# pmgbergen/porepy

Measured on AMD Instinct MI355X. Metric: cells/sec MPFA assemble+solve, 3D unstructured grid, higher is better.
Workload: dtype f64

## Files before the change

### include/porefv.h

```cpp
#ifndef POREFV_H
#define POREFV_H

#include <stddef.h>
#include <stdint.h>

#ifdef __cplusplus
extern "C" {
#endif

typedef struct pfv_ctx pfv_ctx;

typedef enum {
  PFV_OK = 0,
  PFV_ERR_SINGULAR = 1,
  PFV_ERR_CELL_SHAPE = 2,
  PFV_ERR_HIP = 3,
  PFV_ERR_ARGUMENT = 4,
  PFV_ERR_UNSUPPORTED = 5,
  PFV_ERR_NOT_CONVERGED = 6
} pfv_status;

enum {
  PFV_MAT_FLUX = 0,
  PFV_MAT_BOUND_FLUX = 1,
// ... 90 lines not shown
  int64_t sweep_launches;
  double sweep_order_ms;
  int64_t sweep_direct_steps;
  int64_t sweep_direct_fallbacks;
  int64_t transport_multi_components;
  int64_t transport_multi_direct_steps;
  int64_t transport_multi_fallback_components;
  double transport_nl_ms;
  int64_t transport_nl_steps;
  int64_t transport_nl_core_iterations;
  int64_t transport_nl_components;
  double transport_react_ms;
  int64_t transport_react_steps;
  int64_t transport_react_core_iterations;
  int64_t transport_react_components;
  double transport_adjoint_ms;
  int64_t transport_adjoint_steps;
  int64_t transport_adjoint_core_iterations;
  int64_t amg_ap_nnz;
  double transport_react_adjoint_ms;
  int64_t transport_react_adjoint_steps;
  int64_t transport_react_adjoint_core_iterations;
  int64_t amg_galerkin_ap;
} pfv_stats;

pfv_status pfv_create(int device, pfv_ctx** out);
void pfv_destroy(pfv_ctx* h);
const char* pfv_last_error(pfv_ctx* h);
int pfv_is_device_build(void);

pfv_status pfv_set_grid(pfv_ctx* h, int nd, int64_t nc, int64_t nf, int64_t nn,
                        const double* nodes, const int32_t* cf_indptr,
                        const int32_t* cf_indices, const int8_t* cf_sign,
                        const int32_t* fn_indptr, const int32_t* fn_indices,
                        const double* face_normals, const double* face_centers,
                        const double* cell_centers, const double* face_areas);

pfv_status pfv_mpfa_set_params(pfv_ctx* h, const double* perm_33n, const uint8_t* bc_flags,
                               const double* robin_weight, double eta,
                               const double* eta_subface);

pfv_status pfv_mpfa_set_permeability(pfv_ctx* h, const double* perm_33n);

#define PFV_AD_WANT_FLUX_JACOBIAN 1u
pfv_status pfv_mpfa_ad_flux_system(pfv_ctx* h, const double* p, const double* dk_dp, const double* bc_values,
                                   const double* vector_source, const double* source, double* flux_out,
// ... 212 lines not shown
```

### porepy_amd/_lib.py

```python
from __future__ import annotations

import ctypes as C
import os

import numpy as np

_HERE = os.path.dirname(os.path.abspath(__file__))
DEFAULT_LIBRARY = os.path.join(_HERE, "csrc", "libporefv_hip.so")

MAT_FLUX, MAT_BOUND_FLUX, MAT_BOUND_PRESSURE_CELL, MAT_BOUND_PRESSURE_FACE = 0, 1, 2, 3
MAT_VECTOR_SOURCE, MAT_BOUND_PRESSURE_VECTOR_SOURCE, MAT_SYSTEM = 4, 5, 6
MAT_STRESS, MAT_BOUND_STRESS, MAT_BOUND_DISPLACEMENT_CELL, MAT_BOUND_DISPLACEMENT_FACE, MAT_MECH_SYSTEM = 7, 8, 9, 10, 11
MAT_USER_SYSTEM = 12
MAT_FLUX_JACOBIAN = 13
MAT_UPWIND, MAT_UPWIND_RHS_DIR, MAT_UPWIND_RHS_NEU, MAT_TRANSPORT_SYSTEM = 14, 15, 16, 17
MAT_ADVDIFF_SYSTEM = 18
BC_DIR, BC_NEU, BC_ROB, BC_INTERNAL = 1, 2, 4, 8
SOLVE_CG, SOLVE_BICGSTAB, SOLVE_GMRES = 0, 1, 2
PRECOND_JACOBI, PRECOND_AMG, PRECOND_BLOCK, PRECOND_AMG_NNS, PRECOND_SWEEP = 0, 1, 2, 3, 4
FLUXFN_LINEAR, FLUXFN_COREY, FLUXFN_TABLE = 0, 1, 2
DISCR_REBUILD_TOPOLOGY, DISCR_SKIP_VECTOR_SOURCE = 1, 2

STATUS_NAMES = {
    0: "ok", 1: "singular local system", 2: "unsupported cell shape", 3: "HIP error",
# ... 40 lines not shown
                ("win_reused", C.c_int64), ("amg_filter_layout", C.c_int64),
                ("solve_launches", C.c_int64), ("amg_setup_launches", C.c_int64), ("node_redo", C.c_int64),
                ("symbolic_reused", C.c_int64), ("amg_stale_rematches", C.c_int64),
                ("mpsa_contrast_regions", C.c_int64), ("mpsa_max_contrast", C.c_double), ("assemble_positions_kept", C.c_int64),
                ("pipeline_runs", C.c_int64), ("amg_nns_modes", C.c_int64),
                ("face_flux_ms", C.c_double), ("upwind_ms", C.c_double), ("transport_assemble_ms", C.c_double),
                ("transport_advance_ms", C.c_double), ("transport_iterations", C.c_int64),
                ("transport_gmres_retries", C.c_int64),
                ("advdiff_assemble_ms", C.c_double), ("advdiff_advance_ms", C.c_double),
                ("advdiff_iterations", C.c_int64), ("advdiff_precond_fallbacks", C.c_int64),
                ("advdiff_gmres_retries", C.c_int64),
                ("sweep_levels", C.c_int64), ("sweep_core_cells", C.c_int64), ("sweep_launches", C.c_int64),
                ("sweep_order_ms", C.c_double), ("sweep_direct_steps", C.c_int64),
                ("sweep_direct_fallbacks", C.c_int64),
                ("transport_multi_components", C.c_int64), ("transport_multi_direct_steps", C.c_int64),
                ("transport_multi_fallback_components", C.c_int64),
                ("transport_nl_ms", C.c_double), ("transport_nl_steps", C.c_int64),
                ("transport_nl_core_iterations", C.c_int64), ("transport_nl_components", C.c_int64),
                ("transport_react_ms", C.c_double), ("transport_react_steps", C.c_int64),
                ("transport_react_core_iterations", C.c_int64), ("transport_react_components", C.c_int64),
                ("transport_adjoint_ms", C.c_double), ("transport_adjoint_steps", C.c_int64),
                ("transport_adjoint_core_iterations", C.c_int64), ("amg_ap_nnz", C.c_int64),
                ("transport_react_adjoint_ms", C.c_double), ("transport_react_adjoint_steps", C.c_int64),
                ("transport_react_adjoint_core_iterations", C.c_int64), ("amg_galerkin_ap", C.c_int64)]

    def as_dict(self):
        return {n: getattr(self, n) for n, _ in self._fields_}


HALO_FN = C.CFUNCTYPE(C.c_int, C.c_void_p, C.c_void_p, C.c_void_p)
ALLREDUCE_FN = C.CFUNCTYPE(C.c_int, C.c_void_p, C.c_void_p, C.c_int, C.c_void_p)


SENDRECV_FN = C.CFUNCTYPE(C.c_int, C.c_void_p, C.c_int, C.POINTER(C.c_int32), C.c_void_p, C.POINTER(C.c_int64),
                          C.c_void_p, C.POINTER(C.c_int64), C.c_void_p)
ALLGATHER_FN = C.CFUNCTYPE(C.c_int, C.c_void_p, C.c_void_p, C.c_void_p, C.c_int64, C.c_void_p)


class ShardHooks(C.Structure):
    _fields_ = [("exchange_halo", HALO_FN), ("allreduce_sum", ALLREDUCE_FN), ("user", C.c_void_p),
                ("sendrecv", SENDRECV_FN), ("allgather", ALLGATHER_FN)]


class PorefvError(RuntimeError):
    def __init__(self, status: int, message: str):
        super().__init__(f"porefv status {status} ({STATUS_NAMES.get(status, '?')}): {message}")
        self.status = status
# ... 1546 lines not shown
```

### porepy_amd/csrc/amg.inc

```

namespace pfv {

constexpr int kAmgDenseMax = 1024;
constexpr int kAmgCoarseTargetDefault = 160;
constexpr int kAmgMaxLevels = 14;
constexpr int64_t kAmgWTopRows = 600000;
constexpr int kAmgFilterPermilBlock = 50;
constexpr int kAmgFilterPermil = 30;
constexpr int kAmgRounds = 4;
constexpr int kAmgPasses = 3;
constexpr int kAmgGentleCells = 400000;
constexpr int kGalEpl = 8;
constexpr int kGalMaxMembers = 16;
constexpr int64_t kAmgGatherRowsDefault = 32768;

struct AmgSwitches {
  int bs = 1;
  bool omega_auto = false;
  bool safe_rows = true;
  double omega = 0.95, alpha = 1.5;
  int omega_power_steps = 10;
  double omega_sigma = 1.8;
  int passes = kAmgPasses;
  bool passes_coarse_set = false;
  int passes_coarse_raw = -1;
  int rounds = kAmgRounds, rounds_raw = kAmgRounds;
  int strength_neg = 0;
  bool fp32 = true;
  double filter_theta = 0.0;
  int coarse_target = kAmgCoarseTargetDefault;
  bool gamma_set = false;
  int gamma_raw = 0;
  int gamma_levels = 1;
  int64_t fuse_rows = 30000;
  bool fuse_cycle = true;
  bool restrict_lanes = true;
  bool reuse = true, reuse_dist = true, reuse_rebuilt = true;
  int reuse_dist_min_rows = 500000;
  bool members_reuse = true, sizes_reuse = true;
  bool filter_smooth = true, rowmax_reuse = true, filter_layout_reuse = true, skip_moved_digest = true;
  bool galerkin_batched = true, filter_unroll = true, dense_lds = true;
  int64_t gather_rows = kAmgGatherRowsDefault;
  bool post_ap = true;
  bool galerkin_ap = true;
};

static AmgSwitches amg_read_switches(int bs) {
  auto given = [](const char* name, int& v) {
    const char* e = std::getenv(name);
    if (e) v = std::atoi(e);
    return e != nullptr;
  };
  auto on = [](const char* name, int dflt) { return env_int(name, dflt) != 0; };
  AmgSwitches w;
  w.bs = bs;
  w.safe_rows = on("PFV_AMG_SAFE_ROWS", bs == 1 ? 1 : 0);
  int omega_pct = w.safe_rows ? 95 : 80;
  w.omega_auto = !given("PFV_AMG_OMEGA_PCT", omega_pct) && on("PFV_AMG_OMEGA_AUTO", 0);
  w.omega = 0.01 * omega_pct;
  w.alpha = 0.01 * env_int("PFV_AMG_ALPHA_PCT", 150);
  w.omega_power_steps = std::max(2, std::min(30, env_int("PFV_AMG_OMEGA_POWER_STEPS", 10)));
  w.omega_sigma = 0.01 * env_int("PFV_AMG_OMEGA_RHO_PCT", 180);
  w.passes = std::max(1, std::min(6, env_int("PFV_AMG_PASSES", kAmgPasses)));
  w.passes_coarse_set = given("PFV_AMG_PASSES_COARSE", w.passes_coarse_raw);
// ... 1 lines not shown
  w.rounds = std::max(1, std::min(12, w.rounds_raw));
  w.strength_neg = env_int("PFV_AMG_STRENGTH_NEG", 0);
  w.fp32 = on("PFV_AMG_FP32", 1);
  w.filter_theta = 0.001 * env_int(bs == 1 ? "PFV_AMG_FILTER_PERMIL" : "PFV_AMG_FILTER_PERMIL_BLOCK",
                                   bs == 1 ? kAmgFilterPermil : kAmgFilterPermilBlock);
  w.coarse_target = std::max(1, std::min(kAmgDenseMax, env_int("PFV_AMG_COARSE_TARGET", kAmgCoarseTargetDefault)));
  w.gamma_set = given("PFV_AMG_GAMMA", w.gamma_raw);
  w.gamma_levels = env_int("PFV_AMG_GAMMA_LEVELS", 1);
  w.fuse_rows = env_int("PFV_AMG_FUSE_ROWS", 30000);
  w.fuse_cycle = on("PFV_AMG_FUSE_CYCLE", 1);
  w.restrict_lanes = on("PFV_AMG_RESTRICT_LANES", bs == 1 ? 1 : 0);
  w.reuse = on("PFV_AMG_REUSE", 1);
  w.reuse_dist = on("PFV_AMG_REUSE_DIST", 1);
  w.reuse_rebuilt = on("PFV_AMG_REUSE_REBUILT", 1);
  w.reuse_dist_min_rows = env_int("PFV_AMG_REUSE_DIST_MIN_ROWS", 500000);
  w.members_reuse = on("PFV_AMG_MEMBERS_REUSE", 1);
  w.sizes_reuse = on("PFV_AMG_SIZES_REUSE", 1);
  w.filter_smooth = on("PFV_AMG_FILTER_SMOOTH", 1);
  w.rowmax_reuse = on("PFV_AMG_ROWMAX_REUSE", 1);
  w.filter_layout_reuse = on("PFV_AMG_FILTER_LAYOUT_REUSE", 1);
  w.skip_moved_digest = on("PFV_AMG_SKIP_MOVED_DIGEST", 1);
  w.galerkin_batched = on("PFV_AMG_GALERKIN_BATCHED", 1);
  w.filter_unroll = on("PFV_AMG_FILTER_UNROLL", 1);
  w.dense_lds = on("PFV_AMG_DENSE_LDS", 1);
  w.gather_rows = std::max<int64_t>(1, env_int("PFV_AMG_GATHER_ROWS", (int)kAmgGatherRowsDefault));
  w.post_ap = on("PFV_AMG_POST_AP", 1);
  w.galerkin_ap = on("PFV_AMG_GALERKIN_AP", 1);
  return w;
}

static int64_t amg_maps_cfg(const AmgSwitches& w) {
  return ((((int64_t)w.passes * 16 + w.rounds_raw) * 16 + w.passes_coarse_raw + 1) * 4 + w.strength_neg) * 65536 +
         w.coarse_target * 8 + w.bs + (int64_t)(1000.0 * w.filter_theta + 0.5) * (int64_t(1) << 40);
}
static int amg_maps_tag(const AmgSwitches& w) { return w.rounds_raw * 64 + w.passes_coarse_raw + 1; }

struct AmgLevel {
  int64_t n = 0;
  int64_t m = 0;
  const CsrPattern* P = nullptr;
  const double* val = nullptr;
  CsrPattern P_own;
  Buf<double> val_own;
  Buf<float> val32;
  const float* v32 = nullptr;
  WinCsr win_own;
// ... 65 lines not shown
  Amg();
  ~Amg();
  std::unique_ptr<AmgDist> dist;
  bool no_filter = false;
  int64_t finest_cells_parent = 0;
  std::vector<std::unique_ptr<AmgLevel>> lev;
  size_t nlev = 0;
  AmgWork wk;
  int bs = 1;
  AmgSwitches sw;
  int passes = kAmgPasses;
  double omega = 0.8, alpha = 1.5;
  bool omega_auto = true;
  Buf<double> pw_a, pw_b, pw_zero, pw_part;
  Buf<double> dense;
  unsigned long long filt_layout_for = 0;
  bool filt_layout_stable = false;
  CsrPattern filtP;
  Buf<double> filtV;
  double filter_theta = 0.0;
  int64_t filt_nnz = 0;
  bool filter_level0 = false;
  WinCsr filt_win;
  struct GalSizes { int64_t ncr, annz, nnz; int maxcap; };
  std::vector<GalSizes> gal_sizes;
  unsigned long long gal_for_sum = 0;
  bool gal_use = false;
  size_t gal_k = 0;
  int gal_route = 0;
  unsigned long long filt_win_sum = 0;
  bool maps_ok = false, reused = false;
  int64_t maps_n = -1, maps_nnz = -1, maps_cfg = 0;
  unsigned long long maps_sum = 0, maps_epoch = 0;
  int maps_tag = 0;
  int iters_fresh = -1;
  int method_fresh = -1;
  double rtol_fresh = 0.0;
  int64_t stale_rematches = 0;
  void note_iterations(int iterations, double rtol, int method, bool converged) {
    if (!valid) return;
    if (!reused) {
      iters_fresh = converged ? iterations : -1;
      rtol_fresh = rtol;
      method_fresh = method;
    } else if (iters_fresh > 0 && rtol == rtol_fresh && method == method_fresh &&
               (!converged || (double)iterations > 1.3 * (double)iters_fresh + 1.0)) {
// ... 394 lines not shown
  std::swap(a.nnz, b.nnz);
  std::swap(a.max_row, b.max_row);
  a.indptr.swap(b.indptr);
  a.indices.swap(b.indices);
}

static unsigned long long amg_pattern_checksum(pfv_ctx_impl& c, AmgWork& wk, const CsrPattern& P) {
  if (&P == &c.pat_A && c.pat_A_checksum != 0 && c.have_symbolic) return c.pat_A_checksum;
  return read_scalar<unsigned long long>(c.stream, launch_pattern_checksum(c, wk.csum, P));
}

struct AmgBlockStrength {
  const int32_t* ip;
  const double* val;
  int bs;
  PFV_HD double operator()(int64_t r, int kb) const {
    const int64_t i = r / bs;
    double sw = 0.0;
    for (int a = 0; a < bs; ++a) sw += fabs(val[ip[i * bs + a] + kb * bs + a]);
    return sw;
  }
};

#ifndef PFV_EMULATE
constexpr int kFilterUnroll = 5;

static void amg_filter_count_scalar(stream_t s, int64_t n, const int32_t* ip, const int32_t* ix, const double* val,
                                    const double* rmax, double theta, int32_t* cnt) {
  wave_for<16>(s, n, 16, PFV_LAMBDA(const WaveCtx& w) {
    const int64_t r = w.item;
    const int p0 = ip[r], nb = ip[r + 1] - p0;
    const double mi = rmax[r];
    int kept = 0;
    for (int c0 = 0; c0 < nb; c0 += kFilterUnroll * 16) {
      int cj[kFilterUnroll];
      double v[kFilterUnroll], rm[kFilterUnroll];
#pragma unroll
      for (int u = 0; u < kFilterUnroll; ++u) {
        const int kb = c0 + u * 16 + w.lane;
        const bool live = kb < nb;
        cj[u] = live ? ix[p0 + kb] : -1;
        v[u] = live ? val[p0 + kb] : 0.0;
      }
#pragma unroll
      for (int u = 0; u < kFilterUnroll; ++u) rm[u] = cj[u] >= 0 ? rmax[cj[u]] : 0.0;
#pragma unroll
// ... 55 lines not shown
          fv[o] = v[u];
          if (isdiag) { od = o; dv = v[u]; }
        }
        base += total;
      }
    }
    lump[w.lane] = mylump;
    w.lsync();
    if (spec && w.lane0() && base != room) atomic_max_i32(bad, 1);
    const unsigned long long has = __ballot(od >= 0);
    const bool any_diag = ((has >> sh) & 0xffffull) != 0ull;
    if (od >= 0) {
      double sum = 0.0;
      for (int l = 0; l < 16; ++l) sum += lump[l];
      const double d = dv + sum;
      fv[od] = d;
      if (dinv_out) dinv_out[r] = d != 0.0 ? 1.0 / d : 0.0;
    } else if (!any_diag && w.lane0() && dinv_out) {
      dinv_out[r] = 0.0;
    }
    w.lsync();
  });
}
#endif

static void amg_filter(pfv_ctx_impl& c, const AmgSwitches& sw, const CsrPattern& A, const double* val, double theta,
                       CsrPattern& F, Buf<double>& FV, AmgWork& wk, int bs = 1,
                       const std::function<void(double*)>& fill_halo = nullptr, const double* rmax_given = nullptr,
                       double* dinv_out = nullptr, bool same_layout_expected = false, bool* layout_unchanged = nullptr) {
  stream_t s = c.stream;
  const int64_t n = A.nrows;
  const int32_t* ip = A.indptr;
  const int32_t* ix = A.indices;
  int32_t* cnt = wk.cnt.ensure(n + 1);
  int64_t* pos = wk.pos.ensure(n + 2);
  double* rmax = wk.tval.ensure(std::max<int64_t>(std::max(n, A.ncols), 1));
  constexpr int kMaxBs = 4;
  if (bs > kMaxBs) throw Error(PFV_ERR_UNSUPPORTED, "AMG filter: block size above 4");
  const AmgBlockStrength strength{ip, val, bs};
  const bool have_rmax = rmax_given != nullptr && bs == 1 && !fill_halo;
  if (have_rmax) be_d2d(rmax, rmax_given, sizeof(double) * (size_t)n, s);
  else
  wave_for<16>(s, n, 16 * sizeof(double) + 16, PFV_LAMBDA(const WaveCtx& w) {
    const int64_t r = w.item;
    const int64_t i = r / bs;
    double* mx = reinterpret_cast<double*>(w.lds);
    const int p0 = ip[r], nb = (ip[r + 1] - p0) / bs;
    double m = 0.0;
    PFV_LANES(kb, nb) {
      if (ix[p0 + kb * bs] / bs != (int32_t)i) m = fmax(m, strength(r, kb));
    }
    mx[w.lane] = m;
    w.lsync();
    if (w.lane0()) {
      double mm = 0.0;
      for (int l = 0; l < w.width; ++l) mm = fmax(mm, mx[l]);
      rmax[r] = mm;
    }
    w.lsync();
  });
  if (fill_halo) fill_halo(rmax);
  const bool spec = same_layout_expected && F.nrows == n && F.ncols == A.ncols && F.nnz > 0 && F.indptr.p != nullptr;
  int32_t* bad = c.status.ensure(16) + 12;
  if (spec) be_memset(bad, 0, sizeof(int32_t), s);
#ifndef PFV_EMULATE
  const bool fast = bs == 1 && sw.filter_unroll;
#else
  const bool fast = false;
#endif
  if (!spec) {
#ifndef PFV_EMULATE
  if (fast) amg_filter_count_scalar(s, n, ip, ix, val, rmax, theta, cnt);
  else
#endif
  wave_for<16>(s, n, 16 * sizeof(int32_t) + 16, PFV_LAMBDA(const WaveCtx& w) {
    const int64_t r = w.item;
    const int64_t i = r / bs;
    int32_t* ct = reinterpret_cast<int32_t*>(w.lds);
    const int p0 = ip[r], nb = (ip[r + 1] - p0) / bs;
    const double mi = rmax[r];
    int kept = 0;
    PFV_LANES(kb, nb) {
      const int cj = ix[p0 + kb * bs] / bs;
      if (cj == (int32_t)i || strength(r, kb) >= theta * fmin(mi, rmax[(int64_t)cj * bs])) ++kept;
    }
#ifndef PFV_EMULATE
    (void)ct;
    kept += __shfl_xor(kept, 8, 16);
    kept += __shfl_xor(kept, 4, 16);
    kept += __shfl_xor(kept, 2, 16);
    kept += __shfl_xor(kept, 1, 16);
    if (w.lane0()) cnt[r] = kept * bs;
#else
    ct[w.lane] = kept;
    w.lsync();
    if (w.lane0()) {
      int tot = 0;
      for (int l = 0; l < w.width; ++l) tot += ct[l];
      cnt[r] = tot * bs;
    }
    w.lsync();
#endif
  });
  exclusive_scan<int32_t, int64_t>(s, c.scratch, cnt, pos, (size_t)n);
  }
  const bool compare = !spec && layout_unchanged != nullptr && F.nrows == n && F.nnz > 0 && F.indptr.p != nullptr;
  if (!spec) {
    be_memset(pos + n + 1, 0, sizeof(int64_t), s);
    if (compare) {
      const int32_t* old = F.indptr.p;
      parallel_for(s, n, PFV_LAMBDA(int64_t r) {
        if (old[r + 1] - old[r] != cnt[r]) pos[n + 1] = 1;
      });
    }
  }
  int64_t tail[2] = {F.nnz, 0};
  if (!spec) be_d2h(tail, pos + n, 2 * sizeof(int64_t), s);
  if (layout_unchanged) *layout_unchanged = spec || (compare && tail[1] == 0 && tail[0] == F.nnz);
  const int64_t nnz = tail[0];
  F.nrows = n;
  F.ncols = A.ncols;
  F.nnz = nnz;
  F.max_row = A.max_row;
  int32_t* fp = F.indptr.ensure(n + 1);
  int32_t* fx = F.indices.ensure(std::max<int64_t>(nnz, 1));
  double* fv = FV.ensure(std::max<int64_t>(nnz, 1));
  if (!spec) parallel_for(s, n + 1, PFV_LAMBDA(int64_t q) { fp[q] = (int32_t)pos[q]; });
#ifndef PFV_EMULATE
  if (fast) amg_filter_compact_scalar(s, n, ip, ix, val, rmax, theta, fp, fx, fv, dinv_out, spec, bad);
  else
#endif
  wave_for<16>(s, n, (16 + 1) * kMaxBs * sizeof(double) + 20 * sizeof(int32_t) + 16, PFV_LAMBDA(const WaveCtx& w) {
    const int64_t r = w.item;
    const int64_t i = r / bs;
    double* lump = reinterpret_cast<double*>(w.lds);
    double* dblk = lump + 16 * kMaxBs;
    int32_t* flag = reinterpret_cast<int32_t*>(dblk + kMaxBs);
    const int p0 = ip[r], nb = (ip[r + 1] - p0) / bs;
    const double mi = rmax[r];
    if (w.lane0()) flag[16] = -1;
    w.lsync();
    double mylump[kMaxBs];
    for (int b = 0; b < kMaxBs; ++b) mylump[b] = 0.0;
    int base = fp[r];
    for (int c0 = 0; c0 < nb; c0 += w.width) {
      const int kb = c0 + w.lane;
      bool keep = false;
      const bool live = kb < nb;
      bool isdiag = false;
      if (live) {
        const int cj = ix[p0 + kb * bs] / bs;
        isdiag = cj == (int32_t)i;
// ... 36 lines not shown
      base += total * bs;
      w.lsync();
    }
    for (int b = 0; b < bs; ++b) lump[w.lane * kMaxBs + b] = mylump[b];
    w.lsync();
    if (spec && w.lane0() && base != fp[r + 1]) atomic_max_i32(bad, 1);
    if (w.lane0()) {
      const int od = flag[16];
      if (od >= 0) {
        for (int b = 0; b < bs; ++b) {
          double sum = 0.0;
          for (int l = 0; l < w.width; ++l) sum += lump[l * kMaxBs + b];
          const double dv = dblk[b] + sum;
          fv[od + b] = dv;
          if (dinv_out && b == (int)(r - i * bs)) dinv_out[r] = dv != 0.0 ? 1.0 / dv : 0.0;
        }
      } else if (dinv_out) {
        dinv_out[r] = 0.0;
      }
    }
    w.lsync();
  });
  c.stats.amg_filter_layout = spec ? 1 : 0;
  if (spec && read_scalar<int32_t>(s, bad) != 0) {
    amg_filter(c, sw, A, val, theta, F, FV, wk, bs, fill_halo, rmax_given, dinv_out, false, nullptr);
    c.stats.amg_filter_layout = 2;
    if (layout_unchanged) *layout_unchanged = false;
  }
}

static void amg_estimate_omegas(pfv_ctx_impl& c, Amg& amg);
static void amg_build_ap(pfv_ctx_impl& c, Amg& amg, bool want64);
static void amg_spmv(pfv_ctx_impl& c, const Amg& amg, const AmgLevel& L, const double* x, double* y,
                     const double* smooth_b);
static double* amg_cycle(pfv_ctx_impl& c, Amg& amg, size_t l, const double* b, double* x, bool x_is_presmoothed = false,
                         int visit = 0);
static void amg_setup(pfv_ctx_impl& c, Amg& amg, const CsrPattern& A, const double* val, int bs,
                      const double* diag = nullptr, const WinCsr* win0 = nullptr);
static void amg_restrict(pfv_ctx_impl& c, const Amg& amg, const AmgLevel& L, const AmgLevel& Ln, const double* b,
                         const double* t, bool next_smooths);

static void amg_safeguard_rows(pfv_ctx_impl& c, const CsrPattern& P, const double* val, double* dinv) {
  const int32_t* ip = P.indptr;
  const int32_t* ix = P.indices;
  wave_for<16>(c.stream, P.nrows, 16 * sizeof(double) + 16, PFV_LAMBDA(const WaveCtx& w) {
    const int64_t r = w.item;
    double* sh = reinterpret_cast<double*>(w.lds);
    const int p0 = ip[r], len = ip[r + 1] - p0;
    double off = 0.0;
    PFV_LANES(k, len) {
      if (ix[p0 + k] != (int32_t)r) off += fabs(val[p0 + k]);
// ... 117 lines not shown
  parallel_for(s, A.nrows / bs, PFV_LAMBDA(int64_t i) {
    const int len = ip[i * bs + 1] - ip[i * bs];
    bool bad = (len % bs) != 0;
    for (int a = 1; a < bs; ++a) bad = bad || (ip[i * bs + a + 1] - ip[i * bs + a]) != len;
    if (bad) atomic_max_i32(st + 10, 1);
  });
  if (read_scalar<int32_t>(s, st + 10))
    throw Error(PFV_ERR_UNSUPPORTED, "AMG: the matrix is not made of full blocks of the given block size");
}

static unsigned long long amg_setup_level0(pfv_ctx_impl& c, Amg& amg, const CsrPattern& A, const double* val,
                                           const double* diag, const WinCsr* win0, unsigned long long csum) {
  stream_t s = c.stream;
  const AmgSwitches& w = amg.sw;
  AmgDist* D = amg.dist.get();
  const int bs = amg.bs;
  AmgLevel& L0 = amg_level(amg, 0);
  L0.n = A.nrows;
  L0.m = std::max(A.ncols, A.nrows);
  L0.P = &A;
  L0.val = val;
  L0.win = win0;
  amg.filt_nnz = 0;
  amg.filter_level0 = amg.filter_theta > 0.0 && w.filter_smooth;
  if (!amg.filter_level0) {
    double* dv = L0.dinv.ensure(L0.n);
    if (diag) {
      parallel_for(s, L0.n, PFV_LAMBDA(int64_t i) { dv[i] = diag[i] != 0.0 ? 1.0 / diag[i] : 0.0; });
    } else {
      amg_diag_inverse(c, A, val, dv);
    }
    return csum;
  }
  const double* rmax_given = (c.sys_rowmax_for == val && A.nrows == c.nc && w.rowmax_reuse) ? c.sys_rowmax.p : nullptr;
  const bool same_pattern = !D && csum != 0 && amg.filt_layout_for == csum;
  const bool same_layout = same_pattern && amg.filt_layout_stable && w.filter_layout_reuse;
  if (!same_pattern) amg.filtP.nrows = 0;
  bool unchanged = false;
  amg_filter(c, w, A, val, amg.filter_theta, amg.filtP, amg.filtV, amg.wk, bs, amg_fill_halo0(c, D, bs), rmax_given,
             L0.dinv.ensure(L0.n), same_layout, &unchanged);
  amg.filt_layout_stable = unchanged;
  amg.filt_layout_for = D ? 0ull : csum;
  amg.filt_nnz = amg.filtP.nnz;
  L0.P = &amg.filtP;
  L0.val = amg.filtV.p;
  L0.win = nullptr;
  if (amg.filtP.nnz < 200000) return 0ull;
  const bool moved = same_pattern && !unchanged && w.skip_moved_digest;
  const unsigned long long fsum = (env_int("PFV_WIN_REUSE", 1) != 0 && !moved)
                                      ? read_scalar<unsigned long long>(s, launch_pattern_checksum(c, amg.wk.csum, amg.filtP))
                                      : 0ull;
  const bool keep = fsum != 0 && amg.filt_win.ok && amg.filt_win_sum == fsum && amg.filt_win.nrows == amg.filtP.nrows &&
                    amg.filt_win.nnz == amg.filtP.nnz && env_int("PFV_SPMV_WINDOW", 1) != 0;
  if (!keep) {
    if (!(win0 && win_derive(c, amg.filtP, *win0, amg.filt_win))) win_build(c, amg.filtP, amg.filt_win);
    amg.filt_win_sum = amg.filt_win.ok ? fsum : 0ull;
  }
  L0.win = &amg.filt_win;
  return fsum;
}

static void amg_level_buffers(pfv_ctx_impl& c, const Amg& amg, AmgLevel& L, size_t l) {
  if (l > 0) {
    L.x.ensure(L.m);
    L.b.ensure(L.n);
  }
  L.t.ensure(L.m);
  L.v32 = nullptr;
  if (amg.fp32) {
    float* v32 = L.val32.ensure(L.P->nnz);
    const double* v64 = L.val;
    parallel_for(c.stream, L.P->nnz, PFV_LAMBDA(int64_t e) { v32[e] = (float)v64[e]; });
    L.v32 = v32;
  }
  L.nc_cells = 0;
}

static int amg_coarsen_level(pfv_ctx_impl& c, Amg& amg, size_t l, bool reuse) {
  stream_t s = c.stream;
  const AmgSwitches& w = amg.sw;
  AmgWork& wk = amg.wk;
  AmgDist* D = amg.dist.get();
  const int bs = amg.bs;
  AmgLevel& L = *amg.lev[l];
  const int64_t cells = L.n / bs;
  const CsrPattern* curP = L.P;
  const double* curV = L.val;
  if (l == 0 && amg.filter_theta > 0.0 && !amg.filter_level0) {
    amg_filter(c, w, *L.P, L.val, amg.filter_theta, amg.filtP, amg.filtV, wk, bs, amg_fill_halo0(c, D, bs));
    amg.filt_nnz = amg.filtP.nnz;
    curP = &amg.filtP;
    curV = amg.filtV.p;
  }
  int32_t* aggL = L.agg.ensure(cells);
  int64_t cur_cells = cells;
  int slot = -1;
  const int64_t finest_cells = amg.finest_cells_parent > 0 ? amg.finest_cells_parent
                                                            : (D ? D->global_rows0 : amg.lev[0]->n) / bs;
  const int coarse_default = finest_cells >= kAmgGentleCells ? std::min(2, amg.passes) : amg.passes;
  const int passes_here = (l == 0 && amg.finest_cells_parent <= 0)
                              ? amg.passes
                              : std::max(1, std::min(6, w.passes_coarse_set ? w.passes_coarse_raw : coarse_default));
  if (!reuse) L.pmap_count = 0;
  if (!reuse) L.members_kept = false;
  const bool members_reuse = reuse && L.members_kept && w.members_reuse;
  if (l == 0 && !D && members_reuse && L.pmap_count > 0 && w.galerkin_ap && curP == L.P && curV == L.val &&
      !(L.pmap_n[L.pmap_count - 1] > 0.85 * cells)) {
    const int64_t nc = L.pmap_n[L.pmap_count - 1];
    L.nc_cells = nc;
    amg_build_ap(c, amg, true);
    if (amg.ap_ok && amg.ap64_ok) {
      amg_gal_route(amg, 1);
      amg_galerkin_csr(c, w, wk, amg.ap_ptr, amg.ap_col, L.P->nnz, amg.ap_val64, bs, nullptr, L.mptr, L.mem, nc, wk.P[0],
// ... 291 lines not shown
             omega, alpha, x);
  PFV_HIP_CHECK(hipGetLastError());
#endif
}

static void amg_setup_finish(pfv_ctx_impl& c, Amg& amg, const CsrPattern& A, double nnz_sum, unsigned long long csum,
                             unsigned long long level0_sum) {
  const AmgSwitches& w = amg.sw;
  AmgDist* D = amg.dist.get();
  AmgLevel& Lc = *amg.lev[amg.nlev - 1];
  if (D) {
    amg_build_global(c, amg, *D, Lc, *D->plan[amg.nlev - 1]);
  } else if (Lc.n <= kAmgDenseMax) {
    amg.dense_ok = amg_dense_invert(c, w, amg.wk, *Lc.P, Lc.val, amg.dense);
  }
  amg.op_complexity = nnz_sum / (double)A.nnz;
  for (size_t k = 0; k < amg.nlev; ++k) {
    amg.lev[k]->omega = amg.omega;
    amg.lev[k]->rho = 0.0;
  }
  if (w.safe_rows) {
    for (size_t k = 0; k < amg.nlev; ++k) {
      AmgLevel& Lk = *amg.lev[k];
      if (k + 1 < amg.nlev || !amg.dense_ok) amg_safeguard_rows(c, *Lk.P, Lk.val, Lk.dinv);
    }
  }
  if (amg.omega_auto && !D) amg_estimate_omegas(c, amg);
  amg.valid = true;
  if (env_int("PFV_DEBUG_AMG", 0)) {
    std::fprintf(stderr, "amg_setup: filter theta %.3f (nnz %lld -> %lld), levels:", amg.filter_theta, (long long)A.nnz,
                 (long long)amg.filt_nnz);
    for (size_t k = 0; k < amg.nlev; ++k)
      std::fprintf(stderr, " %lld/%lld(w%.3f)", (long long)amg.lev[k]->n, (long long)amg.lev[k]->P->nnz, amg.lev[k]->omega);
    std::fprintf(stderr, " reuse %d\n", (int)amg.reused);
  }
  amg.gal_for_sum = D ? 0ull : level0_sum;
  if (w.reuse && (!D || csum != 0)) {
    amg.maps_ok = true;
    amg.maps_n = A.nrows;
    amg.maps_nnz = A.nnz;
    amg.maps_cfg = amg_maps_cfg(w);
    amg.maps_sum = csum;
    amg.maps_epoch = c.symbolic_epoch;
    amg.maps_tag = amg_maps_tag(w);
  }
}
// ... 636 lines not shown
```

### porepy_amd/csrc/spmv_win.inc

```

namespace pfv {

constexpr int kWinRows = 64;
constexpr int kWinMax = 4096;
constexpr int kWinHash = 8192;

struct SpmvFuse {
  const double* xc = nullptr;
  const double* xc2 = nullptr;
  const int32_t* agg = nullptr;
  int bs = 1;
  double alpha = 0.0;
  double* y2 = nullptr;
};
PFV_HD inline double spmv_prolonged(const SpmvFuse& F, const double* x, int64_t c) {
  const int64_t ci = c / F.bs;
  const int64_t a = (int64_t)F.agg[ci] * F.bs + (c - ci * F.bs);
  double v = F.xc[a];
  if (F.xc2) v += F.xc2[a];
  return x[c] + F.alpha * v;
}

#ifndef PFV_EMULATE
template <bool FILL, bool ONE = false>
// ... 387 lines not shown
    if (env_int("PFV_DEBUG_WIN", 0))
      std::fprintf(stderr, "win_build: rows %lld nnz %lld blocks %lld wmax %d overflow %d\n", (long long)P.nrows,
                   (long long)P.nnz, (long long)nblk, hst[0], hst[1]);
    if (hst[1] != 0) return;
    const int64_t total = read_scalar<int64_t>(s, wptr + nblk);
    int32_t* wcol = W.wcol.ensure(std::max<int64_t>(total, 1));
    uint16_t* lidx = W.lidx.ensure(P.nnz);
    PFV_LAUNCH(HIP_KERNEL_NAME(k_win_build<true>), dim3((unsigned)nblk), dim3(256), 0, s, P.nrows,
                       P.indptr.p, P.indices.p, cnt, wptr, wcol, lidx, st + 12, (int64_t)0);
    PFV_HIP_CHECK(hipGetLastError());
  } else if (env_int("PFV_DEBUG_WIN", 0)) {
    std::fprintf(stderr, "win_build (one pass, stride %lld): rows %lld nnz %lld blocks %lld wmax %d\n", (long long)stride,
                 (long long)P.nrows, (long long)P.nnz, (long long)nblk, hst[0]);
  }
  W.wptr64 = wptr;
  W.nblk = nblk;
  W.nrows = P.nrows;
  W.nnz = P.nnz;
  W.wmax = hst[0];
  W.ok = true;
#endif
}

static bool win_derive(pfv_ctx_impl& c, const CsrPattern& P, const WinCsr& parent, WinCsr& W) {
#ifdef PFV_EMULATE
  (void)c; (void)P; (void)parent; (void)W;
  return false;
#else
  if (!parent.ok || parent.nrows != P.nrows || P.nnz < 1 || env_int("PFV_WIN_DERIVE", 1) == 0) return false;
  const int64_t stride = env_int("PFV_WIN_STRIDE", 1024);
  if (parent.wmax > kWinMax || stride <= 0 || stride > kWinMax) return false;
  stream_t s = c.stream;
  const int64_t nblk = (P.nrows + kWinRows - 1) / kWinRows;
  if (nblk != parent.nblk || (double)nblk * (double)stride * 4.0 > 2.0e9) return false;
  W.ok = false;
  int32_t* cnt = W.cnt.ensure(nblk + 1);
  int64_t* wptr = W.wptr64buf.ensure(nblk + 1);
  int32_t* st = c.status.ensure(16);
  be_memset(st + 12, 0, 2 * sizeof(int32_t), s);
  int32_t* wcol = W.wcol.ensure(std::max<int64_t>(nblk * stride, 1));
  uint16_t* lidx = W.lidx.ensure(P.nnz);
  PFV_LAUNCH(k_win_derive, dim3((unsigned)nblk), dim3(256), 0, s, P.nrows, P.indptr.p, P.indices.p, parent.wptr64,
             parent.wlen, parent.wcol.p, cnt, wptr, wcol, lidx, st + 12, stride);
  PFV_HIP_CHECK(hipGetLastError());
  int32_t hst[2];
  be_d2h(hst, st + 12, sizeof(hst), s);
  if (hst[1] != 0) return false;
  W.wlen = cnt;
  W.wptr64 = wptr;
  W.nblk = nblk;
  W.nrows = P.nrows;
  W.nnz = P.nnz;
  W.wmax = hst[0];
  W.ok = true;
  return true;
#endif
}
// ... 21 lines not shown
```

Baseline: 34.38 million.

## Fuse AMG level-0 strength filter with window build, fp32 copy and safeguard

Adds block-level filter kernels that reuse the level-0 SpMV window (column cache in LDS) to count and compact kept entries. The compact kernel also writes the fp32 values, computes the safeguarded inverse diagonal, and emits the filtered matrix's window layout directly. This removes the separate fp32 conversion, the safeguard pass and the win_derive/win_build launches on level 0. In exchange it adds LDS-capacity checks, a host readback of the per-block maximum kept count, and more complex fallback paths.

```diff
diff --git a/include/porefv.h b/include/porefv.h
--- a/include/porefv.h
+++ b/include/porefv.h
@@ -136,6 +136,7 @@
   int64_t transport_react_adjoint_steps;
   int64_t transport_react_adjoint_core_iterations;
   int64_t amg_galerkin_ap;
+  int64_t amg_filter_block;
 } pfv_stats;
 
 pfv_status pfv_create(int device, pfv_ctx** out);
diff --git a/porepy_amd/_lib.py b/porepy_amd/_lib.py
--- a/porepy_amd/_lib.py
+++ b/porepy_amd/_lib.py
@@ -86,7 +86,8 @@
                 ("transport_adjoint_ms", C.c_double), ("transport_adjoint_steps", C.c_int64),
                 ("transport_adjoint_core_iterations", C.c_int64), ("amg_ap_nnz", C.c_int64),
                 ("transport_react_adjoint_ms", C.c_double), ("transport_react_adjoint_steps", C.c_int64),
-                ("transport_react_adjoint_core_iterations", C.c_int64), ("amg_galerkin_ap", C.c_int64)]
+                ("transport_react_adjoint_core_iterations", C.c_int64), ("amg_galerkin_ap", C.c_int64),
+                ("amg_filter_block", C.c_int64)]
 
     def as_dict(self):
         return {n: getattr(self, n) for n, _ in self._fields_}
diff --git a/porepy_amd/csrc/amg.inc b/porepy_amd/csrc/amg.inc
--- a/porepy_amd/csrc/amg.inc
+++ b/porepy_amd/csrc/amg.inc
@@ -40,6 +40,7 @@
   bool members_reuse = true, sizes_reuse = true;
   bool filter_smooth = true, rowmax_reuse = true, filter_layout_reuse = true, skip_moved_digest = true;
   bool galerkin_batched = true, filter_unroll = true, dense_lds = true;
+  bool filter_block = true;
   int64_t gather_rows = kAmgGatherRowsDefault;
   bool post_ap = true;
   bool galerkin_ap = true;
@@ -87,6 +88,7 @@
   w.skip_moved_digest = on("PFV_AMG_SKIP_MOVED_DIGEST", 1);
   w.galerkin_batched = on("PFV_AMG_GALERKIN_BATCHED", 1);
   w.filter_unroll = on("PFV_AMG_FILTER_UNROLL", 1);
+  w.filter_block = on("PFV_AMG_FILTER_BLOCK", 1);
   w.dense_lds = on("PFV_AMG_DENSE_LDS", 1);
   w.gather_rows = std::max<int64_t>(1, env_int("PFV_AMG_GATHER_ROWS", (int)kAmgGatherRowsDefault));
   w.post_ap = on("PFV_AMG_POST_AP", 1);
@@ -198,6 +200,8 @@
   int64_t filt_nnz = 0;
   bool filter_level0 = false;
   WinCsr filt_win;
+  int64_t filt_blk_max = -1;
+  bool l0_v32_done = false, l0_safeguard_done = false;
   struct GalSizes { int64_t ncr, annz, nnz; int maxcap; };
   std::vector<GalSizes> gal_sizes;
   unsigned long long gal_for_sum = 0;
@@ -638,6 +642,9 @@
   }
 };
 
+constexpr int kFilterBlockCap = 8192;
+constexpr size_t kFilterBlockLds = 56 * 1024;
+
 #ifndef PFV_EMULATE
 constexpr int kFilterUnroll = 5;
 
@@ -739,18 +746,288 @@
     w.lsync();
   });
 }
+
+__global__ void __launch_bounds__(256) k_filter_block_count(int64_t n, const int32_t* __restrict__ ip,
+                                                            const int64_t* __restrict__ wptr,
+                                                            const int32_t* __restrict__ wlen,
+                                                            const int32_t* __restrict__ wcol,
+                                                            const uint16_t* __restrict__ lidx,
+                                                            const double* __restrict__ val,
+                                                            const double* __restrict__ rmax, double theta, int wmax,
+                                                            int32_t* __restrict__ cnt,
+                                                            unsigned long long* __restrict__ blkmax) {
+  extern __shared__ double fb_rms[];
+  int32_t* wcs = reinterpret_cast<int32_t*>(fb_rms + wmax);
+  __shared__ int btot;
+  const int tid = threadIdx.x;
+  const int64_t w0 = wptr[blockIdx.x];
+  const int wn = wlen ? wlen[blockIdx.x] : (int)(wptr[blockIdx.x + 1] - w0);
+  if (tid == 0) btot = 0;
+  for (int i = tid; i < wn; i += 256) {
+    const int32_t cw = wcol[w0 + i];
+    wcs[i] = cw;
+    fb_rms[i] = rmax[cw];
+  }
+  __syncthreads();
+  const int lane = tid & 15;
+  const int64_t row0 = (int64_t)blockIdx.x * kWinRows;
+#pragma unroll 1
+  for (int k = 0; k < kWinRows / 16; ++k) {
+    const int64_t r = row0 + k * 16 + (tid >> 4);
+    if (r >= n) continue;
+    const int p0 = ip[r], nb = ip[r + 1] - p0;
+    const double mi = rmax[r];
+    int kept = 0;
+    for (int c0 = 0; c0 < nb; c0 += kFilterUnroll * 16) {
+      int li[kFilterUnroll];
+      double v[kFilterUnroll];
+#pragma unroll
+      for (int u = 0; u < kFilterUnroll; ++u) {
+        const int kb = c0 + u * 16 + lane;
+        const bool live = kb < nb;
+        li[u] = live ? (int)lidx[p0 + kb] : -1;
+        v[u] = live ? val[p0 + kb] : 0.0;
+      }
+#pragma unroll
+      for (int u = 0; u < kFilterUnroll; ++u)
+        if (li[u] >= 0 && (wcs[li[u]] == (int32_t)r || fabs(v[u]) >= theta * fmin(mi, fb_rms[li[u]]))) ++kept;
+    }
+    kept += __shfl_xor(kept, 8, 16);
+    kept += __shfl_xor(kept, 4, 16);
+    kept += __shfl_xor(kept, 2, 16);
+    kept += __shfl_xor(kept, 1, 16);
+    if (lane == 0) {
+      cnt[r] = kept;
+      atomicAdd(&btot, kept);
+    }
+  }
+  __syncthreads();
+  if (tid == 0) atomicMax(blkmax, (unsigned long long)btot);
+}
+
+struct FilterBlockArgs {
+  int64_t n;
+  const int32_t* ip;
+  const int64_t* wptr;
+  const int32_t* wlen;
+  const int32_t* wcol;
+  const uint16_t* lidx;
+  const double* val;
+  const double* rmax;
+  double theta;
+  int wmax;
+  const int32_t* fp;
+  int32_t* fx;
+  double* fv;
+  float* v32;
+  double* dinv;
+  int safeguard;
+  int spec;
+  int32_t* bad;
+  int emit;
+  int cap;
+  int64_t stride;
+  int32_t* fwcol;
+  int32_t* fwcnt;
+  int64_t* fwptr;
+  uint16_t* flidx;
+  int32_t* fst;
+};
+
+__global__ void __launch_bounds__(256) k_filter_block_main(const FilterBlockArgs a) {
+  extern __shared__ double fb_rms[];
+  int32_t* wcs = reinterpret_cast<int32_t*>(fb_rms + a.wmax);
+  uint16_t* kpos = reinterpret_cast<uint16_t*>(wcs + a.wmax);
+  __shared__ double s_lump[256], s_off[256], s_xch[256];
+  __shared__ unsigned used[kWinMax / 32];
+  __shared__ int wpre[kWinMax / 32 + 1];
+  const int tid = threadIdx.x;
+  const int64_t w0 = a.wptr[blockIdx.x];
+  const int wn = a.wlen ? a.wlen[blockIdx.x] : (int)(a.wptr[blockIdx.x + 1] - w0);
+  for (int i = tid; i < wn; i += 256) {
+    const int32_t cw = a.wcol[w0 + i];
+    wcs[i] = cw;
+    fb_rms[i] = a.rmax[cw];
+  }
+  if (tid < kWinMax / 32) used[tid] = 0u;
+  __syncthreads();
+  const int lane = tid & 15;
+  const int sh = tid & 48;
+  double* lump = s_lump + (tid & ~15);
+  double* offl = s_off + (tid & ~15);
+  double* xch = s_xch + (tid & ~15);
+  const int64_t row0 = (int64_t)blockIdx.x * kWinRows;
+  const int64_t row1 = row0 + kWinRows < a.n ? row0 + kWinRows : a.n;
+  const int fp0 = a.fp[row0];
+  bool over = false;
+#pragma unroll 1
+  for (int k = 0; k < kWinRows / 16; ++k) {
+    const int64_t r = row0 + k * 16 + (tid >> 4);
+    if (r >= a.n) continue;
+    const int p0 = a.ip[r], nb = a.ip[r + 1] - p0;
+    const double mi = a.rmax[r];
+    double mylump = 0.0, myoff = 0.0;
+    const int first = a.fp[r];
+    int base = first;
+    const int room = a.fp[r + 1];
+    int od = -1;
+    double dv = 0.0;
+    for (int c0 = 0; c0 < nb; c0 += kFilterUnroll * 16) {
+      int li[kFilterUnroll], cj[kFilterUnroll];
+      double v[kFilterUnroll], rm[kFilterUnroll];
+#pragma unroll
+      for (int u = 0; u < kFilterUnroll; ++u) {
+        const int kb = c0 + u * 16 + lane;
+        const bool live = kb < nb;
+        li[u] = live ? (int)a.lidx[p0 + kb] : -1;
+        v[u] = live ? a.val[p0 + kb] : 0.0;
+      }
+#pragma unroll
+      for (int u = 0; u < kFilterUnroll; ++u) {
+        cj[u] = li[u] >= 0 ? wcs[li[u]] : -1;
+        rm[u] = li[u] >= 0 ? fb_rms[li[u]] : 0.0;
+      }
+#pragma unroll
+      for (int u = 0; u < kFilterUnroll; ++u) {
+        if (c0 + u * 16 >= nb) break;
+        const bool live = cj[u] >= 0;
+        const bool isdiag = cj[u] == (int32_t)r;
+        bool keep = live && (isdiag || fabs(v[u]) >= a.theta * fmin(mi, rm[u]));
+        if (live && !keep) mylump += v[u];
+        const unsigned long long m = __ballot(keep);
+        const unsigned m16 = (unsigned)((m >> sh) & 0xffffu);
+        const int before = __popc(m16 & ((1u << lane) - 1u));
+        const int total = __popc(m16);
+        if (keep && a.spec && base + before + 1 > room) {
+          atomic_max_i32(a.bad, 1);
+          keep = false;
+        }
+        if (keep) {
+          const int o = base + before;
+          a.fx[o] = cj[u];
+          a.fv[o] = v[u];
+          if (isdiag) { od = o; dv = v[u]; }
+          else if (a.v32) a.v32[o] = (float)v[u];
+          if (a.emit) {
+            atomicOr(&used[li[u] >> 5], 1u << (li[u] & 31));
+            const int q = o - fp0;
+            if (q < a.cap) kpos[q] = (uint16_t)li[u];
+            else over = true;
+          }
+        }
+        if (a.safeguard) {
+          const int qb = base - first;
+          if (keep) xch[(qb + before) & 15] = isdiag ? 0.0 : fabs(v[u]);
+          __builtin_amdgcn_fence(__ATOMIC_SEQ_CST, "wavefront");
+          __builtin_amdgcn_wave_barrier();
+          if (((lane - qb) & 15) < total) myoff += xch[lane];
+          __builtin_amdgcn_fence(__ATOMIC_SEQ_CST, "wavefront");
+          __builtin_amdgcn_wave_barrier();
+        }
+        base += total;
+      }
+    }
+    lump[lane] = mylump;
+    offl[lane] = myoff;
+    __builtin_amdgcn_fence(__ATOMIC_SEQ_CST, "wavefront");
+    __builtin_amdgcn_wave_barrier();
+    if (a.spec && lane == 0 && base != room) atomic_max_i32(a.bad, 1);
+    const unsigned long long has = __ballot(od >= 0);
+    const bool any_diag = ((has >> sh) & 0xffffull) != 0ull;
+    if (od >= 0) {
+      double sum = 0.0;
+      for (int l = 0; l < 16; ++l) sum += lump[l];
+      const double d = dv + sum;
+      a.fv[od] = d;
+      if (a.v32) a.v32[od] = (float)d;
+      if (a.dinv) {
+        double di = d != 0.0 ? 1.0 / d : 0.0;
+        if (a.safeguard) {
+          double off = 0.0;
+          for (int l = 0; l < 16; ++l) off += offl[l];
+          const double ri = off * fabs(di);
+          if (ri > 1.0 && ri < 1.0e300) di = di * 2.0 / (1.0 + ri);
+        }
+        a.dinv[r] = di;
+      }
+    } else if (!any_diag && lane == 0 && a.dinv) {
+      a.dinv[r] = 0.0;
+    }
+    __builtin_amdgcn_fence(__ATOMIC_SEQ_CST, "wavefront");
+    __builtin_amdgcn_wave_barrier();
+  }
+  if (!a.emit) return;
+  if (over) atomicMax(a.fst + 1, 1);
+  __syncthreads();
+  static_assert(kWinMax / 32 == 2 * 64, "one wavefront ranks the mask with two words per lane");
+  if (tid < 64) {
+    const int c0 = __popc(used[2 * tid]), c1 = __popc(used[2 * tid + 1]);
+    int inc = c0 + c1;
+    for (int o = 1; o < 64; o <<= 1) {
+      const int up = __shfl_up(inc, o, 64);
+      if (tid >= o) inc += up;
+    }
+    wpre[2 * tid] = inc - c0 - c1;
+    wpre[2 * tid + 1] = inc - c1;
+    if (tid == 63) wpre[kWinMax / 32] = inc;
+  }
+  __syncthreads();
+  const int total = wpre[kWinMax / 32];
+  const bool fits = total <= a.stride;
+  const int64_t ws0 = (int64_t)blockIdx.x * a.stride;
+  if (tid == 0) {
+    a.fwcnt[blockIdx.x] = total;
+    a.fwptr[blockIdx.x] = ws0;
+    if (!fits) atomicMax(a.fst + 1, 1);
+    else atomicMax(a.fst, total);
+  }
+  if (!fits) return;
+  for (int i = tid; i < wn; i += 256) {
+    const unsigned wd = used[i >> 5];
+    if (wd >> (i & 31) & 1u) a.fwcol[ws0 + wpre[i >> 5] + __popc(wd & ((1u << (i & 31)) - 1u))] = wcs[i];
+  }
+  int nk = a.fp[row1] - fp0;
+  if (nk > a.cap) nk = a.cap;
+  for (int q = tid; q < nk; q += 256) {
+    const int p = kpos[q];
+    const int ps = p < wn ? p : 0;
+    a.flidx[fp0 + q] = (uint16_t)(wpre[ps >> 5] + __popc(used[ps >> 5] & ((1u << (ps & 31)) - 1u)));
+  }
+}
 #endif
+
+constexpr int64_t kAmgWinFromNnz = 200000;
+
+static bool amg_filter_moved(const AmgSwitches& sw, bool same_pattern, bool unchanged) {
+  return same_pattern && !unchanged && sw.skip_moved_digest;
+}
+
+struct AmgFilterBlock {
+  const WinCsr* win0 = nullptr;
+  WinCsr* fwin = nullptr;
+  Buf<float>* v32 = nullptr;
+  bool safeguard = false;
+  bool same_pattern = false;
+  bool win_may_be_kept = false;
+  int64_t win_from_nnz = 0;
+  int64_t win_stride = 0;
+  int64_t* kept_max = nullptr;
+  bool used = false;
+  bool win_emitted = false;
+  bool win_tried = false;
+};
 
 static void amg_filter(pfv_ctx_impl& c, const AmgSwitches& sw, const CsrPattern& A, const double* val, double theta,
                        CsrPattern& F, Buf<double>& FV, AmgWork& wk, int bs = 1,
                        const std::function<void(double*)>& fill_halo = nullptr, const double* rmax_given = nullptr,
-                       double* dinv_out = nullptr, bool same_layout_expected = false, bool* layout_unchanged = nullptr) {
+                       double* dinv_out = nullptr, bool same_layout_expected = false, bool* layout_unchanged = nullptr,
+                       AmgFilterBlock* blk = nullptr) {
   stream_t s = c.stream;
   const int64_t n = A.nrows;
   const int32_t* ip = A.indptr;
   const int32_t* ix = A.indices;
   int32_t* cnt = wk.cnt.ensure(n + 1);
-  int64_t* pos = wk.pos.ensure(n + 2);
+  int64_t* pos = wk.pos.ensure(n + 3);
   double* rmax = wk.tval.ensure(std::max<int64_t>(std::max(n, A.ncols), 1));
   constexpr int kMaxBs = 4;
   if (bs > kMaxBs) throw Error(PFV_ERR_UNSUPPORTED, "AMG filter: block size above 4");
@@ -779,15 +1056,29 @@
   if (fill_halo) fill_halo(rmax);
   const bool spec = same_layout_expected && F.nrows == n && F.ncols == A.ncols && F.nnz > 0 && F.indptr.p != nullptr;
   int32_t* bad = c.status.ensure(16) + 12;
-  if (spec) be_memset(bad, 0, sizeof(int32_t), s);
+  be_memset(bad, 0, 4 * sizeof(int32_t), s);
 #ifndef PFV_EMULATE
   const bool fast = bs == 1 && sw.filter_unroll;
 #else
   const bool fast = false;
 #endif
+  bool block = false;
+#ifndef PFV_EMULATE
+  const WinCsr* W0 = blk ? blk->win0 : nullptr;
+  block = fast && sw.filter_block && !fill_halo && W0 && W0->ok && W0->nrows == n && W0->nnz == A.nnz &&
+          W0->nblk == (n + kWinRows - 1) / kWinRows && W0->wmax >= 1 && W0->wmax <= kWinMax &&
+          (size_t)W0->wmax * 12 <= kFilterBlockLds;
+#endif
+  if (blk) blk->used = blk->win_emitted = blk->win_tried = false;
   if (!spec) {
 #ifndef PFV_EMULATE
-  if (fast) amg_filter_count_scalar(s, n, ip, ix, val, rmax, theta, cnt);
+  if (block) {
+    be_memset(pos + n + 2, 0, sizeof(int64_t), s);
+    PFV_LAUNCH(k_filter_block_count, dim3((unsigned)W0->nblk), dim3(256), (size_t)W0->wmax * 12, s, n, ip, W0->wptr64,
+               W0->wlen, W0->wcol.p, W0->lidx.p, val, rmax, theta, W0->wmax, cnt,
+               reinterpret_cast<unsigned long long*>(pos + n + 2));
+    PFV_HIP_CHECK(hipGetLastError());
+  } else if (fast) amg_filter_count_scalar(s, n, ip, ix, val, rmax, theta, cnt);
   else
 #endif
   wave_for<16>(s, n, 16 * sizeof(int32_t) + 16, PFV_LAMBDA(const WaveCtx& w) {
@@ -831,10 +1122,27 @@
       });
     }
   }
-  int64_t tail[2] = {F.nnz, 0};
-  if (!spec) be_d2h(tail, pos + n, 2 * sizeof(int64_t), s);
-  if (layout_unchanged) *layout_unchanged = spec || (compare && tail[1] == 0 && tail[0] == F.nnz);
+  int64_t tail[3] = {F.nnz, 0, -1};
+  if (!spec) be_d2h(tail, pos + n, (block ? 3 : 2) * sizeof(int64_t), s);
+  const bool unchanged = spec || (compare && tail[1] == 0 && tail[0] == F.nnz);
+  if (layout_unchanged) *layout_unchanged = unchanged;
   const int64_t nnz = tail[0];
+  if (blk && blk->kept_max) {
+    if (!spec) *blk->kept_max = block ? tail[2] : -1;
+    tail[2] = *blk->kept_max;
+  }
+  bool emit = false;
+  int64_t cap = 0;
+  const int64_t wstride = blk ? blk->win_stride : 0;
+  if (block) {
+    const bool moved = amg_filter_moved(sw, blk->same_pattern, unchanged);
+    emit = blk->fwin && wstride > 0 && nnz >= blk->win_from_nnz && (moved || !blk->win_may_be_kept);
+    if (emit) {
+      cap = std::max<int64_t>(tail[2], 1);
+      if (tail[2] < 0 || cap > kFilterBlockCap || (size_t)(blk->win0->wmax) * 12 + (size_t)cap * 2 > kFilterBlockLds)
+        block = emit = false;
+    }
+  }
   F.nrows = n;
   F.ncols = A.ncols;
   F.nnz = nnz;
@@ -844,7 +1152,41 @@
   double* fv = FV.ensure(std::max<int64_t>(nnz, 1));
   if (!spec) parallel_for(s, n + 1, PFV_LAMBDA(int64_t q) { fp[q] = (int32_t)pos[q]; });
 #ifndef PFV_EMULATE
-  if (fast) amg_filter_compact_scalar(s, n, ip, ix, val, rmax, theta, fp, fx, fv, dinv_out, spec, bad);
+  if (block) {
+    FilterBlockArgs a{};
+    a.n = n;
+    a.ip = ip;
+    a.wptr = W0->wptr64;
+    a.wlen = W0->wlen;
+    a.wcol = W0->wcol.p;
+    a.lidx = W0->lidx.p;
+    a.val = val;
+    a.rmax = rmax;
+    a.theta = theta;
+    a.wmax = W0->wmax;
+    a.fp = fp;
+    a.fx = fx;
+    a.fv = fv;
+    a.v32 = blk->v32 ? blk->v32->ensure(std::max<int64_t>(nnz, 1)) : nullptr;
+    a.dinv = dinv_out;
+    a.safeguard = blk->safeguard && dinv_out ? 1 : 0;
+    a.spec = spec ? 1 : 0;
+    a.bad = bad;
+    a.cap = (int)cap;
+    if (emit) {
+      WinCsr* FW = blk->fwin;
+      FW->ok = false;
+      a.emit = 1;
+      a.stride = wstride;
+      a.fwcnt = FW->cnt.ensure(W0->nblk + 1);
+      a.fwptr = FW->wptr64buf.ensure(W0->nblk + 1);
+      a.fwcol = FW->wcol.ensure(std::max<int64_t>(W0->nblk * wstride, 1));
+      a.flidx = FW->lidx.ensure(std::max<int64_t>(nnz, 1));
+      a.fst = bad + 2;
+    }
+    PFV_LAUNCH(k_filter_block_main, dim3((unsigned)W0->nblk), dim3(256), (size_t)W0->wmax * 12 + (size_t)cap * 2, s, a);
+    PFV_HIP_CHECK(hipGetLastError());
+  } else if (fast) amg_filter_compact_scalar(s, n, ip, ix, val, rmax, theta, fp, fx, fv, dinv_out, spec, bad);
   else
 #endif
   wave_for<16>(s, n, (16 + 1) * kMaxBs * sizeof(double) + 20 * sizeof(int32_t) + 16, PFV_LAMBDA(const WaveCtx& w) {
@@ -927,11 +1269,32 @@
     w.lsync();
   });
   c.stats.amg_filter_layout = spec ? 1 : 0;
-  if (spec && read_scalar<int32_t>(s, bad) != 0) {
-    amg_filter(c, sw, A, val, theta, F, FV, wk, bs, fill_halo, rmax_given, dinv_out, false, nullptr);
+  int32_t flags[4] = {0, 0, 0, 0};
+  if (emit) be_d2h(flags, bad, sizeof(flags), s);
+  else if (spec) flags[0] = read_scalar<int32_t>(s, bad);
+  if (spec && flags[0] != 0) {
+    amg_filter(c, sw, A, val, theta, F, FV, wk, bs, fill_halo, rmax_given, dinv_out, false, nullptr, blk);
     c.stats.amg_filter_layout = 2;
     if (layout_unchanged) *layout_unchanged = false;
-  }
+    return;
+  }
+  if (blk) {
+    blk->used = block;
+    blk->win_tried = emit;
+  }
+#ifndef PFV_EMULATE
+  if (emit && flags[3] == 0) {
+    WinCsr& FW = *blk->fwin;
+    FW.wlen = FW.cnt.p;
+    FW.wptr64 = FW.wptr64buf.p;
+    FW.nblk = W0->nblk;
+    FW.nrows = n;
+    FW.nnz = nnz;
+    FW.wmax = flags[2];
+    FW.ok = true;
+    blk->win_emitted = true;
+  }
+#endif
 }
 
 static void amg_estimate_omegas(pfv_ctx_impl& c, Amg& amg);
@@ -1095,6 +1458,8 @@
   L0.val = val;
   L0.win = win0;
   amg.filt_nnz = 0;
+  amg.l0_v32_done = amg.l0_safeguard_done = false;
+  c.stats.amg_filter_block = 0;
   amg.filter_level0 = amg.filter_theta > 0.0 && w.filter_smooth;
   if (!amg.filter_level0) {
     double* dv = L0.dinv.ensure(L0.n);
@@ -1110,23 +1475,44 @@
   const bool same_layout = same_pattern && amg.filt_layout_stable && w.filter_layout_reuse;
   if (!same_pattern) amg.filtP.nrows = 0;
   bool unchanged = false;
+  AmgFilterBlock fb;
+  const bool offer_block = bs == 1 && !D && win0 && win0->ok && w.filter_block;
+  if (offer_block) {
+    fb.win0 = win0;
+    fb.fwin = &amg.filt_win;
+    fb.v32 = amg.fp32 ? &L0.val32 : nullptr;
+    fb.safeguard = w.safe_rows && A.nrows > kAmgDenseMax;
+    fb.same_pattern = same_pattern;
+    fb.win_may_be_kept = amg.filt_win.ok && env_int("PFV_WIN_REUSE", 1) != 0;
+    fb.win_from_nnz = kAmgWinFromNnz;
+    fb.win_stride = win_derived_stride(*win0, A.nrows);
+    fb.kept_max = &amg.filt_blk_max;
+  } else {
+    amg.filt_blk_max = -1;
+  }
   amg_filter(c, w, A, val, amg.filter_theta, amg.filtP, amg.filtV, amg.wk, bs, amg_fill_halo0(c, D, bs), rmax_given,
-             L0.dinv.ensure(L0.n), same_layout, &unchanged);
+             L0.dinv.ensure(L0.n), same_layout, &unchanged, offer_block ? &fb : nullptr);
+  amg.l0_v32_done = fb.used && fb.v32 != nullptr;
+  amg.l0_safeguard_done = fb.used && fb.safeguard;
+  c.stats.amg_filter_block = fb.used ? (fb.win_emitted ? 2 : 1) : 0;
   amg.filt_layout_stable = unchanged;
   amg.filt_layout_for = D ? 0ull : csum;
   amg.filt_nnz = amg.filtP.nnz;
   L0.P = &amg.filtP;
   L0.val = amg.filtV.p;
   L0.win = nullptr;
-  if (amg.filtP.nnz < 200000) return 0ull;
-  const bool moved = same_pattern && !unchanged && w.skip_moved_digest;
+  if (amg.filtP.nnz < kAmgWinFromNnz) return 0ull;
+  const bool moved = amg_filter_moved(w, same_pattern, unchanged);
   const unsigned long long fsum = (env_int("PFV_WIN_REUSE", 1) != 0 && !moved)
                                       ? read_scalar<unsigned long long>(s, launch_pattern_checksum(c, amg.wk.csum, amg.filtP))
                                       : 0ull;
-  const bool keep = fsum != 0 && amg.filt_win.ok && amg.filt_win_sum == fsum && amg.filt_win.nrows == amg.filtP.nrows &&
-                    amg.filt_win.nnz == amg.filtP.nnz && env_int("PFV_SPMV_WINDOW", 1) != 0;
-  if (!keep) {
-    if (!(win0 && win_derive(c, amg.filtP, *win0, amg.filt_win))) win_build(c, amg.filtP, amg.filt_win);
+  const bool keep = !fb.win_tried && fsum != 0 && amg.filt_win.ok && amg.filt_win_sum == fsum &&
+                    amg.filt_win.nrows == amg.filtP.nrows && amg.filt_win.nnz == amg.filtP.nnz &&
+                    env_int("PFV_SPMV_WINDOW", 1) != 0;
+  if (fb.win_emitted) {
+    amg.filt_win_sum = fsum;
+  } else if (!keep) {
+    if (!(win0 && !fb.win_tried && win_derive(c, amg.filtP, *win0, amg.filt_win))) win_build(c, amg.filtP, amg.filt_win);
     amg.filt_win_sum = amg.filt_win.ok ? fsum : 0ull;
   }
   L0.win = &amg.filt_win;
@@ -1143,7 +1529,7 @@
   if (amg.fp32) {
     float* v32 = L.val32.ensure(L.P->nnz);
     const double* v64 = L.val;
-    parallel_for(c.stream, L.P->nnz, PFV_LAMBDA(int64_t e) { v32[e] = (float)v64[e]; });
+    if (!(l == 0 && amg.l0_v32_done)) parallel_for(c.stream, L.P->nnz, PFV_LAMBDA(int64_t e) { v32[e] = (float)v64[e]; });
     L.v32 = v32;
   }
   L.nc_cells = 0;
@@ -1162,6 +1548,7 @@
   if (l == 0 && amg.filter_theta > 0.0 && !amg.filter_level0) {
     amg_filter(c, w, *L.P, L.val, amg.filter_theta, amg.filtP, amg.filtV, wk, bs, amg_fill_halo0(c, D, bs));
     amg.filt_nnz = amg.filtP.nnz;
+    amg.filt_blk_max = -1;
     curP = &amg.filtP;
     curV = amg.filtV.p;
   }
@@ -1499,6 +1886,7 @@
   if (w.safe_rows) {
     for (size_t k = 0; k < amg.nlev; ++k) {
       AmgLevel& Lk = *amg.lev[k];
+      if (k == 0 && amg.l0_safeguard_done) continue;
       if (k + 1 < amg.nlev || !amg.dense_ok) amg_safeguard_rows(c, *Lk.P, Lk.val, Lk.dinv);
     }
   }
diff --git a/porepy_amd/csrc/spmv_win.inc b/porepy_amd/csrc/spmv_win.inc
--- a/porepy_amd/csrc/spmv_win.inc
+++ b/porepy_amd/csrc/spmv_win.inc
@@ -433,17 +433,24 @@
 #endif
 }
 
+static int64_t win_derived_stride(const WinCsr& parent, int64_t nrows) {
+  if (!parent.ok || parent.nrows != nrows || env_int("PFV_WIN_DERIVE", 1) == 0) return 0;
+  const int64_t stride = env_int("PFV_WIN_STRIDE", 1024);
+  if (parent.wmax > kWinMax || stride <= 0 || stride > kWinMax) return 0;
+  const int64_t nblk = (nrows + kWinRows - 1) / kWinRows;
+  if (nblk != parent.nblk || (double)nblk * (double)stride * 4.0 > 2.0e9) return 0;
+  return stride;
+}
+
 static bool win_derive(pfv_ctx_impl& c, const CsrPattern& P, const WinCsr& parent, WinCsr& W) {
 #ifdef PFV_EMULATE
   (void)c; (void)P; (void)parent; (void)W;
   return false;
 #else
-  if (!parent.ok || parent.nrows != P.nrows || P.nnz < 1 || env_int("PFV_WIN_DERIVE", 1) == 0) return false;
-  const int64_t stride = env_int("PFV_WIN_STRIDE", 1024);
-  if (parent.wmax > kWinMax || stride <= 0 || stride > kWinMax) return false;
+  const int64_t stride = P.nnz < 1 ? 0 : win_derived_stride(parent, P.nrows);
+  if (stride == 0) return false;
   stream_t s = c.stream;
   const int64_t nblk = (P.nrows + kWinRows - 1) / kWinRows;
-  if (nblk != parent.nblk || (double)nblk * (double)stride * 4.0 > 2.0e9) return false;
   W.ok = false;
   int32_t* cnt = W.cnt.ensure(nblk + 1);
   int64_t* wptr = W.wptr64buf.ensure(nblk + 1);
```

Result: faster. 34.73 million, median of 6 (+1.0%).
